# owl-project/owlExaBrick

Measured on AMD Instinct MI355X. Metric: frames/sec at 2048^2 DVR, exajet-like, MI355X, higher is better.
Workload: dtype f32; 1 GPU; c4_exajet (seed 0xe7a0003 procedural AMR, scale 1.0): 640512000 cells / 1251000 bricks / 13349488 regions, 2048x2048 DVR, dt 0.5, alpha ramp, gradient shading on, space skipping on, frameID 0; tiling=16x16 tiles interleaved over 1 GPU(s)

## Files before the change

### owlexabrick_amd/csrc/exa_device.h

```cpp
#pragma once
#include "../../include/exa_hip.h"
#include <hip/hip_runtime.h>

#include <vector>

#ifndef EXA_MARCH_WAVES
#define EXA_MARCH_WAVES 6
#endif
#ifndef EXA_ROPE_WAVES
#define EXA_ROPE_WAVES 7
#endif
#ifndef EXA_MULTI_WAVES
#define EXA_MULTI_WAVES 6
#endif
#ifndef EXA_PREPASS_WAVES
#define EXA_PREPASS_WAVES 4
#endif
#ifndef EXA_IL2_WAVES
#define EXA_IL2_WAVES 5
#endif
#ifndef EXA_IL34_WAVES
#define EXA_IL34_WAVES 4
#endif
#ifndef EXA_PREPASS_ISO_WAVES
#define EXA_PREPASS_ISO_WAVES 4
#endif
#ifndef EXA_AO_ISO_WAVES
#define EXA_AO_ISO_WAVES 6
#endif
#ifndef EXA_EMPTY_CELLS
#define EXA_EMPTY_CELLS 0
#endif
#ifndef EXA_BASIS_FORM
#define EXA_BASIS_FORM 0
#endif
namespace exa {

struct alignas(64) BvhNode {
  float4 q0, q1, q2;
  int32_t child0, child1, pad0, pad1;
};
static_assert(sizeof(BvhNode) == 64, "node must be one 64-byte line");

struct alignas(16) RegionInfo {
  int32_t listBegin;
  int32_t listSize;
  float   finestLevelCellWidth;
  int32_t firstBrick;
};

struct alignas(16) KdNodeDev {
  float    split;
  uint32_t word;
  int32_t  left, right;
};
static_assert(sizeof(KdNodeDev) == 16, "kd node = one 16-byte load");

struct alignas(16) RopeLeaf {
  float    lo[3], hi0;
  float    hi1, hi2;
  uint32_t rec;
  uint32_t flags;
  int32_t  rope[6];
  int32_t  region;
  int32_t  pad;
};
static_assert(sizeof(RopeLeaf) == 64, "rope leaf = four 16-byte loads");

struct alignas(16) RegionRec {
  float   lo[3], hi0;
  float   hi1, hi2, finestLevelCellWidth; int32_t firstBrick;
  int32_t listBegin, listSize, pad0, pad1;
};
static_assert(sizeof(RegionRec) == 48, "region record = three 16-byte loads");

struct DeviceScene {
  const int4       *bricks;
  const int32_t    *leafList;
  const int4       *leafHdr;
  const float      *scalars;
  const RegionInfo *regionInfo;
  const float2     *valueRange;
  const float      *domain;
  unsigned long long channelOffset[EXA_MAX_CHANNELS];
  uint32_t numRegions;
  uint32_t numInternal;
};

#ifndef EXA_KD_STACK
#define EXA_KD_STACK 4
#endif
#ifndef EXA_KD_STACK_MULTI
#define EXA_KD_STACK_MULTI 3
#endif
#ifndef EXA_ROPE_QUEUE
#define EXA_ROPE_QUEUE 5
#endif
#ifndef EXA_ROPE_QUEUE_MULTI
#define EXA_ROPE_QUEUE_MULTI 5
#endif
#ifndef EXA_SEG_QUEUE
#define EXA_SEG_QUEUE 4
#endif
enum { kKdStackEntries = EXA_KD_STACK, kKdStackMultiEntries = EXA_KD_STACK_MULTI };
enum { kTile = 16, kTilePixels = 256, kStackDepth = 32, kKdStack = EXA_KD_STACK, kKdStackMulti = EXA_KD_STACK_MULTI, kSegQueue = EXA_SEG_QUEUE,
       kRopeQueue = EXA_ROPE_QUEUE, kRopeQueueMulti = EXA_ROPE_QUEUE_MULTI,
       kKdBlock = 256,
       kWideSegCap = 256,
       kWalkProbeBits = 15, kWalkProbeSize = 1 << kWalkProbeBits };

enum StatSlot { ST_SEGMENTS, ST_SAMPLE_EVALS, ST_SAMPLES, ST_BRICK_VISITS, ST_CORNER_LOADS,
                ST_ISO_SEGMENTS, ST_ISO_EVALS, ST_NODES,
                ST_W_BRICK, ST_L_BRICK, ST_W_FINAL, ST_L_FINAL, ST_W_NODE, ST_L_NODE, ST_W_LEAF, ST_L_LEAF,
                ST_KD_MISMATCH,
                ST_T_BRICK, ST_T_FINAL, ST_T_WALK, ST_T_SEG, ST_T_OTHER,
                ST_RESTARTS, ST_UNION, ST_PROBE_OVERFLOW, ST_WAVE_ITERS, ST_TILE_ITERS,
                ST_ROPE_LEAVES,
                ST_COUNT };

struct alignas(16) AoRecord { float4 posFd, ngAmb, baseRnd; uint32_t slot, pad0, pad1, pad2; };
static_assert(sizeof(AoRecord) == 64, "AO record = four 16-byte stores");

struct RenderArgs {
  DeviceScene        sc;
  const BvhNode     *volNodes;
  const BvhNode     *isoNodes;
  const KdNodeDev   *kdNodes;
  const KdNodeDev   *kdMarchNodes;
  int32_t            kdMarchRoot;
  uint32_t           leafBeginBits, leafSizeBits;
  const RegionRec   *regionRec;
  const RopeLeaf    *ropeLeaves;
  const KdNodeDev   *ropeNodes;
  int32_t            ropeRoot;
  int32_t            ropeFastDiv;
  int32_t            ropeAddr32;
  int32_t            kdRoot;
  int32_t            kdIsoRoot;
  float              kdLo[3], kdHi[3];
  const BvhNode     *meshNodes;
  const float       *meshVerts;
  const int32_t     *meshTris;
  int32_t            numTris;
  const BvhNode     *streamNodes;
  const float       *traces;
  int32_t            numStreamPrims;
  int32_t            tracerChannels[3], numTraces, numTimesteps, timestep;
  float              steplen;
  float              worldLo[3], worldHi[3];
  ExaHipFrameState   fs;
  ExaHipParams       p;
  const float4      *xf;
  const float       *cellsIl;
  int32_t            il32;
  int32_t            mul24;
  int32_t            addr32;
  float              invDtPow2;
  int32_t            fastSampler;
  float              tfFracMagic;
  int32_t            numXfChannels;
  int32_t            W, H, tilesX, tilesY;
  int32_t            rank, world;
  const int32_t     *tileMap;
  uint32_t          *color;
  int32_t            colorRowMajor;
  float4            *accum;
  float4            *surf;
  float4            *pixOut;
  uint32_t          *surfRnd;
  unsigned long long *stats;
  int32_t           *errorFlag;
  int32_t            debugPixel;
  const int32_t     *wideTileMap;
  float4            *wideSegs;
  uint32_t          *walkProbe;
  AoRecord          *aoRecs;
  uint32_t          *aoCount;
  uint32_t          *aoKeys;
  uint32_t          *aoHist;
  uint32_t          *aoOrder;
  uint8_t           *aoHit;
  uint32_t           aoBins;
  uint32_t          *tileCostPre;
  uint32_t          *tileCost;
};

struct SampleArgs {
  const int4        *leafHdr;
  const float       *scalars;
  const KdNodeDev   *kdNodes;
  const RegionRec   *regionRec;
  int32_t            kdRoot;
  int32_t            maxSteps;
  float              kdLo[3], kdHi[3];
  int32_t           *errorFlag;
  int32_t            world;
  int32_t            normalized;
  float              fill;
  ExaHipFrameState   fs;
  int32_t            numChannels;
  unsigned long long fieldOffset[EXA_MAX_CHANNELS];
  const float       *points;
  unsigned long long count;
  float             *values, *gradients;
  int32_t           *status;
  float              lo[3], step[3];
  int32_t            box0[3], box1[3];
  unsigned long long patchesX, patchesY, numPatches;
  unsigned long long strideY, strideZ;
  float             *out;
};
enum { kSamplePatchShapes = 4 };

hipError_t buildLbvhTopologyDevice(const float *boxes, uint32_t numPrims, BvhNode *nodes, int32_t *levelIds,
                                   std::vector<uint32_t> &internalNodesPerDepth, hipStream_t s);

#define EXA_FORM_LAUNCHERS                                                                                              \
  hipError_t launchRender(const RenderArgs &a, int numBlocks, bool grad, bool iso, bool stats, hipStream_t s);          \
  hipError_t launchSurfacePrepassKd(const RenderArgs &a, int numBlocks, bool stats, hipStream_t s);                     \
   \
  hipError_t launchAoRaysKd(const RenderArgs &a, int numBlocks, hipStream_t s);                                         \
  hipError_t launchCompositeKd(const RenderArgs &a, int numBlocks, hipStream_t s);                                      \
  hipError_t launchRenderKd(const RenderArgs &a, int numBlocks, bool grad, bool fast, bool surf,                        \
                            int stats , hipStream_t s);                                 \
                                                                    \
  hipError_t launchRenderKdRope(const RenderArgs &a, int numBlocks, bool grad, bool fast, bool surf,                    \
                                int stats, hipStream_t s);                                                              \
  hipError_t launchRenderKdWide(const RenderArgs &a, int numTiles, int lanesPerRay, bool grad, bool fast, bool surf,    \
                                hipStream_t s);                                                                         \
                          \
  hipError_t launchComputeTraces(const RenderArgs &a, float *traces, int count, hipStream_t s);                        \
    \
  hipError_t launchSamplePoints(const SampleArgs &a, bool grad, hipStream_t s);                                      \
  hipError_t launchSampleGrid(const SampleArgs &a, int shape, bool uniform, hipStream_t s);
namespace form0 { EXA_FORM_LAUNCHERS }
namespace form1 { EXA_FORM_LAUNCHERS }
namespace form0e { EXA_FORM_LAUNCHERS }
#undef EXA_FORM_LAUNCHERS

hipError_t launchVolumeActivity(const DeviceScene &sc, const ExaHipFrameState &fs, const ExaHipParams &p,
                                const float4 *xf, uint8_t *active, float tfFracMagic, hipStream_t s);
hipError_t launchIsoActivity(const DeviceScene &sc, const ExaHipFrameState &fs, uint8_t *active, hipStream_t s);
hipError_t launchRefit(BvhNode *nodes, const int32_t *nodeIds, int count, const float *domain,
                       const uint8_t *active, hipStream_t s);
hipError_t launchKdRefit(KdNodeDev *nodes, KdNodeDev *marchNodes, const int32_t *nodeIds, int count, const uint8_t *active, int which, hipStream_t s);
hipError_t launchRopeActivity(RopeLeaf *leaves, uint32_t numRegions, const uint8_t *active, int which, uint32_t *activeCount, hipStream_t s);
hipError_t launchPermuteBricks(const float *src, float *dst, const uint32_t *srcBegin, const uint32_t *dstBegin, int4 *bricks,
                               unsigned long long numBricks, int4 *leafHdr, const int32_t *leafList, unsigned long long leafListSize,
                               unsigned long long totalCells, int numFields, hipStream_t s);
hipError_t launchInterleave(const DeviceScene &sc, unsigned long long totalCells, int nch, float *out, hipStream_t s);
hipError_t launchUntile(const uint32_t *gathered, unsigned long long shardStride, int world,
                        int W, int H, uint32_t *out, hipStream_t s);
hipError_t launchProfileMarker(int tag, hipStream_t s);

}
```

### owlexabrick_amd/csrc/exa_kernels.hip

```cpp
#include "exa_device.h"
#include <cfloat>

#if EXA_BASIS_FORM == 0 && EXA_EMPTY_CELLS
#define EXA_FORM_NS form0e
#elif EXA_BASIS_FORM == 0
#define EXA_FORM_NS form0
#elif EXA_BASIS_FORM == 1 && EXA_EMPTY_CELLS
#error "empty cells are a per-corner property: the per-axis association (EXA_BASIS_FORM 1) does not apply"
#elif EXA_BASIS_FORM == 1
#define EXA_FORM_NS form1
#else
#error "EXA_BASIS_FORM is 0 (source order) or 1 (per-axis association with fused multiply-adds)"
#endif
#define EXA_F1 (EXA_BASIS_FORM == 1)
#ifndef EXA_TU_ROPE
#define EXA_TU_ROPE 0
#endif
#ifndef EXA_TU_SAMPLE
#define EXA_TU_SAMPLE 0
#endif
namespace exa {
namespace EXA_FORM_NS {

struct V3 { float x, y, z; };
// ... 1595 lines not shown
  if (!ISO_ONLY && C.a->numTris > 0) traceMeshes(C, ray, prd);
  if (!ISO_ONLY && withContourPlanes) {
    for (int i = 0; i < EXA_MAX_CONTOUR_PLANES; ++i)
      if (C.a->fs.contour[i].enabled) {
        auto find = [&](V3 pos) { return kdFindRegion(C, pos, stackF, qRegion, qT); };
        const SurfaceHit c = traceContourRay(C, ray, mk(C.a->fs.contour[i].normal), C.a->fs.contour[i].offset,
                                             C.a->fs.contour[i].channel, find);
        if (c.primID == EXA_PRIMID_PLANE && c.t_hit < prd.t_hit) prd = c;
      }
  }
  if (!ISO_ONLY && C.a->numStreamPrims > 0) traceStreamlines(C, ray, prd);
  bool activeIso = false;
  for (int i = 0; i < EXA_MAX_ISO_SURFACES; i++) activeIso |= (C.a->fs.iso[i].enabled != 0);
  if (activeIso) {
    const SurfaceHit isoPRD = traceIsoRayKd(C, ray, 0.f, stackF, qRegion, qT, !withContourPlanes);
    if (isoPRD.primID == EXA_PRIMID_ISOSURFACE && isoPRD.t_hit < prd.t_hit) prd = isoPRD;
  }
}

template <int STATS, bool ISO_ONLY, bool AO_DEFER>
__global__ __launch_bounds__(kKdBlock, (ISO_ONLY ? EXA_PREPASS_ISO_WAVES : EXA_PREPASS_WAVES)) void surfacePrepassKdKernel(const RenderArgs a)
{
  extern __shared__ __attribute__((aligned(16))) unsigned char smem[];
  float4 *xfLds = reinterpret_cast<float4 *>(smem);
  unsigned char *sp0 = smem + size_t(a.numXfChannels) * EXA_NUM_XF_VALUES * sizeof(float4);
  int *stackRef = reinterpret_cast<int *>(sp0);
  float *stackF = reinterpret_cast<float *>(sp0 + size_t(kKdStackEntries) * kKdBlock * 4) + threadIdx.x;
  int *qRegion = reinterpret_cast<int *>(sp0 + size_t(kKdStack) * kKdBlock * 12) + threadIdx.x;
  float *qT = reinterpret_cast<float *>(sp0 + size_t(kKdStack) * kKdBlock * 12 + size_t(kSegQueue) * kKdBlock * 4) + threadIdx.x;
  for (int i = threadIdx.x; i < a.numXfChannels * EXA_NUM_XF_VALUES; i += kKdBlock) xfLds[i] = a.xf[i];
  __syncthreads();

  Ctx<STATS> C;
  C.a = &a;
  C.xfLds = xfLds;
  C.stack = stackRef + threadIdx.x;
  C.guardTripped = false;
  C.fastSampler = a.fastSampler != 0 && STATS != 1;
  if (STATS) for (int i = 0; i < ST_COUNT; i++) C.st[i] = 0;

  const int wavesPerBlock = kKdBlock / 64;
  const int gwave = blockIdx.x * wavesPerBlock + (threadIdx.x >> 6);
  const int tile = a.tileMap[gwave >> 2];
  const int tx = tile % a.tilesX, ty = tile / a.tilesX;
  const int wave = gwave & 3, lane = threadIdx.x & 63;
  const int inX = ((wave & 1) << 3) + laneX(lane), inY = ((wave >> 1) << 3) + laneY(lane);
  const int px = tx * kTile + inX, py = ty * kTile + inY;
  const bool inside = px < a.W && py < a.H && (a.debugPixel < 0 || a.debugPixel == px + a.W * py);

  if (inside) {
    const ExaHipFrameState &fs = a.fs;
    const int frameID = fs.frameID;
    Lcg rnd;
    rnd.init((uint32_t)(frameID * a.W * a.H) + (uint32_t)px, (uint32_t)py);
    const float sx = float(px) + rnd.next();
    const float sy = float(py) + rnd.next();
    Ray ray;
    ray.org = mk(fs.cam_pos);
    ray.dir = normalize((mk(fs.cam_dir00) + sx * mk(fs.cam_dirDu)) + sy * mk(fs.cam_dirDv));
    ray.tmin = 1e-6f; ray.tmax = 1e8f;
    V3 bgColor = mk(0.f, 0.f, 0.f);
    float surface_t_hit = ray.tmax;
    bool deferAo = false;
    AoRecord rec;
    {
      SurfaceHit surface;
      traceSurfacesKd<STATS, ISO_ONLY>(C, ray, surface, true, stackF, qRegion, qT);
      surface_t_hit = surface.t_hit;
      if (surface.primID >= 0 || surface.primID == EXA_PRIMID_ISOSURFACE || surface.primID == EXA_PRIMID_PLANE
          || surface.primID == EXA_PRIMID_STREAMLINE) {
        const bool shade = surface.primID >= 0 || surface.primID == EXA_PRIMID_PLANE || surface.primID == EXA_PRIMID_STREAMLINE
                        || (surface.primID == EXA_PRIMID_ISOSURFACE && a.p.gradientShadingISO);
        if (AO_DEFER && shade && length(surface.Ng) > 0.f && fs.ao.enabled) {
          const V3 isect_pos = ray.org + surface.t_hit * ray.dir;
          rec.posFd = make_float4(isect_pos.x, isect_pos.y, isect_pos.z, fabsf(dot(ray.dir, surface.Ng)));
          rec.ngAmb = make_float4(surface.Ng.x, surface.Ng.y, surface.Ng.z, surface.ambient);
          rec.baseRnd = make_float4(surface.baseColor.x, surface.baseColor.y, surface.baseColor.z, __uint_as_float(rnd.state));
          rnd.next(); rnd.next(); rnd.next(); rnd.next();
          deferAo = true;
        } else if (shade && length(surface.Ng) > 0.f) {
          const float AO_Radius = fs.ao.length;
          const int AO_Samples = (!AO_DEFER && fs.ao.enabled) ? 2 : 0;
          const V3 isect_pos = ray.org + surface.t_hit * ray.dir;
          const V3 wN = surface.Ng;
          const V3 vN = fabsf(wN.x) > fabsf(wN.y) ? normalize(mk(-wN.z, 0.f, wN.x)) : normalize(mk(0.f, wN.z, -wN.y));
          const V3 uN = cross(vN, wN);
          int hitCnt = 0;
          for (int i = 0; i < AO_Samples; ++i) {
            const float u1 = rnd.next(), u2 = rnd.next();
            const float r = sqrtf(u1);
            const float theta = 2.f * 3.14159265358979323846f * u2;
            const V3 sp = mk(r * cosf(theta), r * sinf(theta), sqrtf(1.f - u1));
            Ray ao_ray;
            ao_ray.org = isect_pos;
            ao_ray.dir = normalize((sp.x * uN + sp.y * vN) + sp.z * wN);
            ao_ray.tmin = 1e-4f; ao_ray.tmax = AO_Radius;
            SurfaceHit ao;
            traceSurfacesKd<STATS, ISO_ONLY>(C, ao_ray, ao, false, stackF, qRegion, qT);
            if (ao.primID >= 0 || ao.primID == EXA_PRIMID_ISOSURFACE || ao.primID == EXA_PRIMID_PLANE
                || ao.primID == EXA_PRIMID_STREAMLINE) hitCnt++;
          }
          const float shadow = (!AO_DEFER && fs.ao.enabled) ? (float)hitCnt / AO_Samples : 0.f;
          const float fd = fabsf(dot(ray.dir, surface.Ng));
          const float ns = 1.f - shadow;
          bgColor = mk(surface.ambient + surface.baseColor.x * fd * ns,
                       surface.ambient + surface.baseColor.y * fd * ns,
                       surface.ambient + surface.baseColor.z * fd * ns);
        } else {
          bgColor = surface.baseColor;
        }
      }
    }
    const size_t slot = (a.world == 1) ? size_t(px) + size_t(a.W) * py
                                       : size_t(tile / a.world) * kTilePixels + (inY * kTile + inX);
    a.surf[slot] = make_float4(bgColor.x, bgColor.y, bgColor.z, surface_t_hit);
    a.surfRnd[slot] = rnd.state;
    if (AO_DEFER) {
      const unsigned long long m = __ballot(deferAo);
      if (m) {
        const int lane_ = threadIdx.x & 63;
        const int leader = __ffsll((long long)m) - 1;
        unsigned base = 0;
        if (lane_ == leader) base = atomicAdd(a.aoCount, (unsigned)__popcll(m));
        base = (unsigned)__shfl((int)base, leader, 64);
        if (deferAo) {
          rec.slot = (uint32_t)slot; rec.pad0 = rec.pad1 = rec.pad2 = 0;
          a.aoRecs[base + (unsigned)__popcll(m & ((1ull << lane_) - 1ull))] = rec;
        }
      }
    }
  }

  if (a.tileCostPre) {
    unsigned v = inside ? C.isoSteps : 0u;
    for (int off = 32; off > 0; off >>= 1) v = max(v, (unsigned)__shfl_down((int)v, off, 64));
    if ((threadIdx.x & 63) == 0) atomicMax(&a.tileCostPre[tile], v);
  }
  if (C.guardTripped) atomicExch(a.errorFlag, 1);
  if (STATS) {
    for (int i = 0; i < ST_COUNT; i++) {
      unsigned long long v = inside ? C.st[i] : 0ull;
      for (int off = 32; off > 0; off >>= 1) v += __shfl_down(v, off, 64);
      if ((threadIdx.x & 63) == 0 && v) atomicAdd(&a.stats[i], v);
    }
  }
}

__device__ __forceinline__ Ray aoRayOf(const ExaHipFrameState &fs, const float4 posFd, const float4 ngAmb, const float4 baseRnd, unsigned j)
{
  Lcg rnd;
  rnd.state = __float_as_uint(baseRnd.w);
  if (j & 1u) { rnd.next(); rnd.next(); }
  const V3 wN = mk(ngAmb.x, ngAmb.y, ngAmb.z);
  const V3 vN = fabsf(wN.x) > fabsf(wN.y) ? normalize(mk(-wN.z, 0.f, wN.x)) : normalize(mk(0.f, wN.z, -wN.y));
  const V3 uN = cross(vN, wN);
  const float u1 = rnd.next(), u2 = rnd.next();
  const float rr = sqrtf(u1);
  const float theta = 2.f * 3.14159265358979323846f * u2;
  const V3 sp = mk(rr * cosf(theta), rr * sinf(theta), sqrtf(1.f - u1));
  Ray ao_ray;
  ao_ray.org = mk(posFd.x, posFd.y, posFd.z);
  ao_ray.dir = normalize((sp.x * uN + sp.y * vN) + sp.z * wN);
  ao_ray.tmin = 1e-4f; ao_ray.tmax = fs.ao.length;
  return ao_ray;
}

enum { kAoDirClasses = 24, kAoCellShift = 5 };
__device__ __forceinline__ uint32_t aoRayKey(const RenderArgs &a, uint32_t slot, V3 d)
{
  const float ax = fabsf(d.x), ay = fabsf(d.y), az = fabsf(d.z);
  const uint32_t dom = (ax >= ay && ax >= az) ? 0u : (ay >= az ? 1u : 2u);
  const uint32_t oct = (d.x < 0.f ? 1u : 0u) | (d.y < 0.f ? 2u : 0u) | (d.z < 0.f ? 4u : 0u);
  uint32_t cell;
  if (a.world == 1) {
    const uint32_t px = slot % (uint32_t)a.W, py = slot / (uint32_t)a.W;
    cell = (py >> kAoCellShift) * (((uint32_t)a.W + 31u) >> kAoCellShift) + (px >> kAoCellShift);
  } else {
    cell = slot >> 10;
  }
  return cell * kAoDirClasses + oct * 3u + dom;
}
#if !EXA_TU_ROPE
__global__ __launch_bounds__(256) void aoKeyKernel(const RenderArgs a)
{
  const unsigned numRays = 2u * a.aoCount[0];
  for (unsigned j = blockIdx.x * 256u + threadIdx.x; j < numRays; j += gridDim.x * 256u) {
    const AoRecord *r = a.aoRecs + (j >> 1);
    const Ray ray = aoRayOf(a.fs, r->posFd, r->ngAmb, r->baseRnd, j);
    const uint32_t key = min(aoRayKey(a, r->slot, ray.dir), a.aoBins - 1u);
    a.aoKeys[j] = key;
    atomicAdd(&a.aoHist[key], 1u);
  }
}
__global__ __launch_bounds__(1024) void aoScanKernel(uint32_t *hist, uint32_t numBins)
{
  __shared__ uint32_t part[1024];
  const uint32_t per = (numBins + 1023u) / 1024u;
  const uint32_t b0 = min(threadIdx.x * per, numBins), b1 = min(b0 + per, numBins);
  uint32_t sum = 0;
  for (uint32_t b = b0; b < b1; b++) sum += hist[b];
  part[threadIdx.x] = sum;
  __syncthreads();
  for (uint32_t off = 1; off < 1024u; off <<= 1) {
    const uint32_t v = threadIdx.x >= off ? part[threadIdx.x - off] : 0u;
    __syncthreads();
    part[threadIdx.x] += v;
    __syncthreads();
  }
  uint32_t run = part[threadIdx.x] - sum;
  for (uint32_t b = b0; b < b1; b++) { const uint32_t c = hist[b]; hist[b] = run; run += c; }
}
__global__ __launch_bounds__(256) void aoScatterKernel(const RenderArgs a)
{
  const unsigned numRays = 2u * a.aoCount[0];
  for (unsigned j = blockIdx.x * 256u + threadIdx.x; j < numRays; j += gridDim.x * 256u)
    a.aoOrder[atomicAdd(&a.aoHist[a.aoKeys[j]], 1u)] = j;
}
__global__ __launch_bounds__(256) void aoFinalizeKernel(const RenderArgs a)
{
  const unsigned numHits = a.aoCount[0];
  for (unsigned h = blockIdx.x * 256u + threadIdx.x; h < numHits; h += gridDim.x * 256u) {
    const AoRecord *r = a.aoRecs + h;
    const float4 posFd = r->posFd, ngAmb = r->ngAmb, baseRnd = r->baseRnd;
    const uint32_t slot = r->slot;
    const int hitCnt = (int)a.aoHit[2u * h] + (int)a.aoHit[2u * h + 1u];
    const float shadow = (float)hitCnt / 2;
    const float fd = posFd.w;
    const float ns = 1.f - shadow;
    const float t_hit = a.surf[slot].w;
    a.surf[slot] = make_float4(ngAmb.w + baseRnd.x * fd * ns, ngAmb.w + baseRnd.y * fd * ns, ngAmb.w + baseRnd.z * fd * ns, t_hit);
  }
}

#endif

template <bool ISO_ONLY, bool SORTED>
__global__ __launch_bounds__(kKdBlock, (ISO_ONLY ? EXA_AO_ISO_WAVES : EXA_PREPASS_WAVES)) void aoRaysKdKernel(const RenderArgs a)
{
  extern __shared__ __attribute__((aligned(16))) unsigned char smem[];
  float4 *xfLds = reinterpret_cast<float4 *>(smem);
  unsigned char *sp0 = smem + size_t(a.numXfChannels) * EXA_NUM_XF_VALUES * sizeof(float4);
  int *stackRef = reinterpret_cast<int *>(sp0);
  float *stackF = reinterpret_cast<float *>(sp0 + size_t(kKdStackEntries) * kKdBlock * 4) + threadIdx.x;
  int *qRegion = reinterpret_cast<int *>(sp0 + size_t(kKdStack) * kKdBlock * 12) + threadIdx.x;
  float *qT = reinterpret_cast<float *>(sp0 + size_t(kKdStack) * kKdBlock * 12 + size_t(kSegQueue) * kKdBlock * 4) + threadIdx.x;
  for (int i = threadIdx.x; i < a.numXfChannels * EXA_NUM_XF_VALUES; i += kKdBlock) xfLds[i] = a.xf[i];
  __syncthreads();
  Ctx<0> C;
  C.a = &a;
  C.xfLds = xfLds;
  C.stack = stackRef + threadIdx.x;
  C.guardTripped = false;
  C.fastSampler = a.fastSampler != 0;
  const ExaHipFrameState &fs = a.fs;
  const unsigned numRays = 2u * a.aoCount[0];
  for (;;) {
    unsigned base = 0;
    if ((threadIdx.x & 63) == 0) base = atomicAdd(&a.aoCount[2], 64u);
    base = (unsigned)__shfl((int)base, 0, 64);
    if (base >= numRays) break;
    const unsigned k = base + (threadIdx.x & 63);
    const bool live = k < numRays;
    const unsigned j = (SORTED && live) ? a.aoOrder[k] : k;
    int hitFlag = 0;
    float4 posFd = make_float4(0.f, 0.f, 0.f, 0.f), ngAmb = posFd, baseRnd = posFd;
    uint32_t slot = 0;
    if (live) {
      const AoRecord *r = a.aoRecs + (j >> 1);
      posFd = r->posFd; ngAmb = r->ngAmb; baseRnd = r->baseRnd; slot = r->slot;
      const Ray ao_ray = aoRayOf(fs, posFd, ngAmb, baseRnd, j);
      SurfaceHit ao;
      traceSurfacesKd<0, ISO_ONLY>(C, ao_ray, ao, false, stackF, qRegion, qT);
      if (ao.primID >= 0 || ao.primID == EXA_PRIMID_ISOSURFACE || ao.primID == EXA_PRIMID_PLANE
          || ao.primID == EXA_PRIMID_STREAMLINE) hitFlag = 1;
      if (SORTED) a.aoHit[j] = (uint8_t)hitFlag;
    }
    if (SORTED) continue;
    const int other = __shfl_xor(hitFlag, 1, 64);
    if (live && !(j & 1u)) {
      const int hitCnt = hitFlag + other;
      const float shadow = (float)hitCnt / 2;
      const float fd = posFd.w;
      const float ns = 1.f - shadow;
      const float t_hit = a.surf[slot].w;
      a.surf[slot] = make_float4(ngAmb.w + baseRnd.x * fd * ns, ngAmb.w + baseRnd.y * fd * ns, ngAmb.w + baseRnd.z * fd * ns, t_hit);
    }
  }
  if (C.guardTripped) atomicExch(a.errorFlag, 1);
}

constexpr int marchWaves(int MULTI, int STATS, bool SMALL, int NCH, bool ROPE)
{
  return NCH ? (NCH == 2 ? EXA_IL2_WAVES : EXA_IL34_WAVES)
             : (MULTI == 1 ? EXA_MULTI_WAVES
                           : (MULTI ? 5 : ((ROPE && !STATS && SMALL && EXA_BASIS_FORM == 1) ? EXA_ROPE_WAVES : EXA_MARCH_WAVES)));
}

template <bool GRAD, bool FAST, int MULTI, bool SURF, int STATS, bool SMALL, int NCH = 0, bool ROPE = false>
__global__ __launch_bounds__(kKdBlock, marchWaves(MULTI, STATS, SMALL, NCH, ROPE)) void renderFrameKdKernel(const RenderArgs a)
{
  constexpr bool LEAN = marchWaves(MULTI, STATS, SMALL, NCH, ROPE) >= 7;
  constexpr int PACKED_CT = !ROPE ? -1 : (STATS == 1 ? 0 : (SMALL ? 1 : -1));
  const bool packedRec = PACKED_CT < 0 ? a.leafBeginBits != 0 : PACKED_CT != 0;
  static_assert(NCH == 0 || (MULTI == 2 && STATS == 0), "the interleaved march is a multi-channel variant of the shipped kernel");
  constexpr int KSB = MULTI == 1 ? kKdStackMulti : kKdStack;
  constexpr int KS = MULTI == 1 ? kKdStackMultiEntries : kKdStackEntries;
  constexpr int QN = ROPE ? (MULTI == 1 ? kRopeQueueMulti : kRopeQueue) : kSegQueue;
  static_assert(MULTI != 0 || (size_t(EXA_NUM_XF_VALUES) * sizeof(float4) + size_t(kKdBlock) * (ROPE ? QN * 16 : (KSB + QN) * 12))
                                  * marchWaves(MULTI, STATS, SMALL, NCH, ROPE) <= 160 * 1024,
                "LDS per workgroup x waves per SIMD exceeds the CU's 160 KB: shorten the queue or lower the occupancy");
  extern __shared__ __attribute__((aligned(16))) unsigned char smem[];
  float4 *xfLds = reinterpret_cast<float4 *>(smem);
  unsigned char *sp0 = smem + size_t(a.numXfChannels) * EXA_NUM_XF_VALUES * sizeof(float4);
  int *stackRef = reinterpret_cast<int *>(sp0);
  float *stackF = reinterpret_cast<float *>(sp0 + size_t(KS) * kKdBlock * 4) + threadIdx.x;
  unsigned char *q0 = ROPE ? sp0 : sp0 + size_t(KSB) * kKdBlock * 12;
  int *qRegion = reinterpret_cast<int *>(q0) + threadIdx.x;
  float *qT = reinterpret_cast<float *>(q0 + size_t(QN) * kKdBlock * 4) + threadIdx.x;
  float4 *queue4 = reinterpret_cast<float4 *>(sp0) + threadIdx.x;
  for (int i = threadIdx.x; i < a.numXfChannels * EXA_NUM_XF_VALUES; i += kKdBlock) xfLds[i] = a.xf[i];
  __syncthreads();

  Ctx<STATS> C;
  C.a = &a;
  C.xfLds = xfLds;
  C.stack = stackRef + threadIdx.x;
  C.guardTripped = false;
  const unsigned long long clockBegin = clock64();
  if (STATS) for (int i = 0; i < ST_COUNT; i++) C.st[i] = 0;
  __shared__ unsigned long long lapMarks[STATS == 2 ? 8 * (kKdBlock / 64) : 1];
  if (STATS == 2) {
    C.lapMark = lapMarks + 8 * (threadIdx.x >> 6);
    if ((threadIdx.x & 63) == 0) {
      C.lapMark[0] = clock64(); C.lapMark[1] = ST_T_OTHER - ST_T_BRICK;
      for (int i = 2; i < 7; i++) C.lapMark[i] = 0;
    }
  }

  const int wavesPerBlock = kKdBlock / 64;
  const int gwave = blockIdx.x * wavesPerBlock + (threadIdx.x >> 6);
  const int tile = a.tileMap[gwave >> 2];
  const int tx = tile % a.tilesX, ty = tile / a.tilesX;
  const int wave = gwave & 3, lane = threadIdx.x & 63;
  const int inX = ((wave & 1) << 3) + laneX(lane), inY = ((wave >> 1) << 3) + laneY(lane);
  const int px = tx * kTile + inX, py = ty * kTile + inY;
  const bool inside = px < a.W && py < a.H && (a.debugPixel < 0 || a.debugPixel == px + a.W * py);

  if (STATS == 1 && a.walkProbe) C.probe = a.walkProbe + size_t(gwave) * kWalkProbeSize;
  unsigned marchIters = 0;
  if (inside) {
    const ExaHipFrameState &fs = a.fs;
    const int frameID = fs.frameID;
    Lcg rnd;
    rnd.init((uint32_t)(frameID * a.W * a.H) + (uint32_t)px, (uint32_t)py);
    const float sx = float(px) + rnd.next();
    const float sy = float(py) + rnd.next();
    Ray ray;
    ray.org = mk(fs.cam_pos);
    ray.dir = normalize((mk(fs.cam_dir00) + sx * mk(fs.cam_dirDu)) + sy * mk(fs.cam_dirDv));
    ray.tmin = 1e-6f; ray.tmax = 1e8f;
    float surface_t_hit = ray.tmax;
    if (SURF) {
      const size_t slot0 = (a.world == 1) ? size_t(px) + size_t(a.W) * py
                                          : size_t(tile / a.world) * kTilePixels + (inY * kTile + inX);
      surface_t_hit = a.surf[slot0].w;
      rnd.state = a.surfRnd[slot0];
    }
    const float interleavedSamplingOffset = rnd.next();
    ray.tmax = surface_t_hit;
    if (fs.clipBox.enabled) {
      float c0, c1;
      boxTest(ray, mk(fs.clipBox.lo), mk(fs.clipBox.hi), c0, c1);
      ray.tmin = c0; ray.tmax = c1;
    }
    surface_t_hit = ray.tmax;
    ray.org = xfmPoint(fs, ray.org);
    ray.org.x = __int_as_float(__builtin_amdgcn_readfirstlane(__float_as_int(ray.org.x)));
    ray.org.y = __int_as_float(__builtin_amdgcn_readfirstlane(__float_as_int(ray.org.y)));
    ray.org.z = __int_as_float(__builtin_amdgcn_readfirstlane(__float_as_int(ray.org.z)));
    ray.dir = xfmVector(fs, ray.dir);
    const float dt_scale = length(ray.dir);
    ray.dir = normalize(ray.dir);
    ray.tmin = dt_scale * ray.tmin;
    ray.tmax = surface_t_hit * dt_scale;

    Color4 pixelColor; pixelColor.x = pixelColor.y = pixelColor.z = pixelColor.w = 0.f;
    const int numChannels = a.p.numPrimaryChannels;

    KdWalk w;
    w.pk.v = 0;
    {
      Ray whole = ray; whole.tmin = -INFINITY; whole.tmax = INFINITY;
      float r0, r1;
      const bool hit = boxTest(whole, mk(a.kdLo), mk(a.kdHi), r0, r1);
      w.tn = fmaxf(r0, ray.tmin);
      w.tf = fminf(r1, ray.tmax);
      w.tEnd = w.tf;
      w.ref = (hit && w.tn < w.tf) ? (ROPE ? a.ropeRoot : a.kdMarchRoot) : EXA_KD_DONE;
    }
    bool ropeFast = false;
    if (ROPE) ropeFast = a.ropeFastDiv != 0 && !anyLane(!ropeRayInRange(ray));

    float walkTmin = ray.tmin;

    bool haveSeg = false;
    int listBegin = 0, listSize = 0;
    float flcw = 1.f;
    float t1 = 0.f, t_i = 0.f, t_sample = 0.f, actual_dt = 0.f;
    int child = 0, chan = 0;
    int4 hb0 = make_int4(0, 0, 0, 1), hb1 = make_int4(1, 1, 1, 0);
    Basis B;
    B.sumWV = 0.f; B.sumW = 0.f; B.sumD = mk(0.f, 0.f, 0.f); B.sumDC = mk(0.f, 0.f, 0.f);
    float xWV[NCH > 1 ? NCH - 1 : 1];
    V3 xD[NCH > 1 ? NCH - 1 : 1];
#pragma unroll
    for (int c = 0; c < (NCH > 1 ? NCH - 1 : 1); c++) { xWV[c] = 0.f; xD[c] = mk(0.f, 0.f, 0.f); }
    const float *field0 = a.sc.scalars + a.sc.channelOffset[0];
    const float *field = field0;
    float xfRcpRange0 = 0.f, xfRange0 = 0.f;
    if (FAST && !MULTI) {
      xfRange0 = __int_as_float(__builtin_amdgcn_readfirstlane(__float_as_int((fs.xfDomain[0][1] - fs.xfDomain[0][0]) + 1e-20f)));
      xfRcpRange0 = __int_as_float(__builtin_amdgcn_readfirstlane(__float_as_int(__builtin_amdgcn_rcpf(xfRange0))));
    }
    float xfRcpRangeN[NCH ? NCH : 1], xfRangeN[NCH ? NCH : 1];
#pragma unroll
    for (int c = 0; c < (NCH ? NCH : 1); c++) {
      xfRangeN[c] = (FAST && NCH) ? __int_as_float(__builtin_amdgcn_readfirstlane(__float_as_int((fs.xfDomain[c][1] - fs.xfDomain[c][0]) + 1e-20f))) : 0.f;
      xfRcpRangeN[c] = (FAST && NCH) ? __int_as_float(__builtin_amdgcn_readfirstlane(__float_as_int(__builtin_amdgcn_rcpf(xfRangeN[c])))) : 0.f;
    }

    unsigned iter = 0;
    for (;; iter++) {
      if (iter == 0xfffffff0u) { C.guardTripped = true; break; }
      if (anyLane(!haveSeg && w.pk.get(PK_QCOUNT) == 0 && w.ref != EXA_KD_DONE)) {
        C.lap(ST_T_WALK);
        do {
          const bool want = w.pk.get(PK_QCOUNT) < QN && w.ref != EXA_KD_DONE;
          if (want) {
            if (ROPE) ropeStep<STATS, SMALL, QN, LEAN, PACKED_CT>(C, w, walkTmin, a, queue4, ray, ropeFast, interleavedSamplingOffset);
            else kdStep<false, STATS, SMALL, KS>(C, w, walkTmin, a, stackF, qRegion, qT, ray, 0, walkTmin, 1.f, a.kdMarchNodes, a.kdMarchRoot);
          }
        } while (anyLane(!haveSeg && w.pk.get(PK_QCOUNT) == 0 && w.ref != EXA_KD_DONE));
      }
      if (!haveSeg) {
        C.lap(ST_T_SEG);
        const int qc = w.pk.get(PK_QCOUNT);
        if (qc == 0) break;
        const int qh = w.pk.get(PK_QHEAD);
        int region;
        float t0, tiQueued = 0.f;
        if (ROPE) {
          const float4 e = queue4[qh * kKdBlock];
          region = __float_as_int(e.x); t1 = e.y; tiQueued = e.z; t0 = e.w;
        } else {
          region = qRegion[qh * kKdBlock];
          t0 = qT[(2 * qh) * kKdBlock];
          t1 = qT[(2 * qh + 1) * kKdBlock];
        }
        w.pk.template incWrap<QN>(PK_QHEAD);
        w.pk.dec(PK_QCOUNT);
        if (packedRec) {
          const unsigned d = (unsigned)region;
          listBegin = (int)(d & ((1u << a.leafBeginBits) - 1u));
          listSize = (int)((d >> a.leafBeginBits) & ((1u << a.leafSizeBits) - 1u)) + 1;
          flcw = __int_as_float((127 + (int)(d >> (a.leafBeginBits + a.leafSizeBits))) << 23);
        } else {
          const RegionInfo ri = a.sc.regionInfo[region];
          listBegin = ri.listBegin; listSize = ri.listSize;
          flcw = ri.finestLevelCellWidth;
        }
        C.count(ST_SEGMENTS);
        haveSeg = true;
        w.pk.setBit(PK_NEEDHDR);
        if (ROPE && packedRec)
          t_i = tiQueued;
        else if (a.invDtPow2 != 0.f)
          t_i = firstSampleTPow2(t0, a.p.dt * flcw, a.invDtPow2 * __int_as_float(0x7f000000 - __float_as_int(flcw)), interleavedSamplingOffset);
        else
          t_i = firstSampleT(t0, a.p.dt * flcw, interleavedSamplingOffset);
        {
          const float t_next = fminf(t_i, t1);
          t_sample = 0.5f * (fminf(t1, t_next) + t0);
          actual_dt = t_next - t0;
        }
        C.count(ST_SAMPLE_EVALS);
      }

      C.lap(ST_T_BRICK);
      C.phase(ST_W_BRICK);
      if (listSize > 1 || w.pk.get(PK_NEEDHDR)) {
        if (SMALL) {
          const char *hp = reinterpret_cast<const char *>(a.sc.leafHdr) + ((uint32_t)(listBegin + child) << 5);
          hb0 = *reinterpret_cast<const int4 *>(hp); hb1 = *reinterpret_cast<const int4 *>(hp + 16);
        } else {
          const unsigned at = 2u * (unsigned)(listBegin + child);
          hb0 = a.sc.leafHdr[at]; hb1 = a.sc.leafHdr[at + 1u];
        }
        w.pk.clearField(PK_NEEDHDR);
      }
      if (NCH) addBasisFastIl<GRAD, SMALL, (NCH ? NCH : 2)>(B, xWV, xD, hb0, hb1, a.cellsIl, rayAt(ray.org, t_sample, ray.dir));
      else addBasisFast<GRAD, STATS, SMALL>(C, B, hb0, hb1, MULTI ? field : field0, rayAt(ray.org, t_sample, ray.dir));
      child++;
      if (child < listSize) continue;

      C.lap(ST_T_FINAL);
      C.phase(ST_W_FINAL);
      if (NCH) {
        if (B.sumW > 1e-20f) {
#pragma unroll
          for (int c = 0; c < NCH; c++) {
            const float wv = c == 0 ? B.sumWV : xWV[c == 0 ? 0 : c - 1];
            const V3 sd = c == 0 ? B.sumD : xD[c == 0 ? 0 : c - 1];
            const float cellValue = fdivExact<FAST>(wv, B.sumW);
            V3 grad = mk(0.f, 0.f, 0.f);
            if (GRAD) grad = gradOf(B.sumW, wv, sd, B.sumDC);
            integrateVolume<FAST, STATS, FAST>(C, ray, pixelColor, actual_dt, cellValue, grad, flcw, c, xfRcpRangeN[c], xfRangeN[c]);
          }
        }
#pragma unroll
        for (int c = 0; c < (NCH > 1 ? NCH - 1 : 1); c++) { xWV[c] = 0.f; xD[c] = mk(0.f, 0.f, 0.f); }
      } else if (B.sumW > 1e-20f) {
        C.count(ST_SAMPLES);
        const float cellValue = fdivExact<FAST>(B.sumWV, B.sumW);
        V3 grad = mk(0.f, 0.f, 0.f);
        if (GRAD) grad = gradOf(B.sumW, B.sumWV, B.sumD, B.sumDC);
        integrateVolume<FAST, STATS, (FAST && !MULTI), LEAN>(C, ray, pixelColor, actual_dt, cellValue, grad, flcw, MULTI ? chan : 0, xfRcpRange0, xfRange0);
      }
      B.sumWV = 0.f; B.sumW = 0.f; B.sumD = mk(0.f, 0.f, 0.f); B.sumDC = mk(0.f, 0.f, 0.f);
      child = 0;
      if (MULTI && !NCH) {
        chan++;
        if (chan < numChannels) {
          field = a.sc.scalars + a.sc.channelOffset[chan];
          C.count(ST_SAMPLE_EVALS);
          continue;
        }
        chan = 0; field = field0;
      }
      if (pixelColor.w >= EXA_TERMINATION_THRESHOLD) {
        pixelColor.x = pixelColor.x * pixelColor.w;
        pixelColor.y = pixelColor.y * pixelColor.w;
        pixelColor.z = pixelColor.z * pixelColor.w;
        pixelColor.w = 1.f;
        break;
      }
      const float t_last = fminf(t_i, t1);
      if (t_last >= t1) {
        haveSeg = false;
        continue;
      }
      t_i += a.p.dt * flcw;
      {
        const float t_next = fminf(t_i, t1);
        t_sample = 0.5f * (fminf(t1, t_next) + t_last);
        actual_dt = t_next - t_last;
      }
      C.count(ST_SAMPLE_EVALS);
    }

    C.lap(ST_T_OTHER);
    marchIters = iter;
    size_t slot, colorSlot;
    {
      unsigned tid = threadIdx.x, bid = blockIdx.x;
      asm volatile("" : "+v"(tid));
      asm volatile("" : "+s"(bid));
      const int lane2 = tid & 63, wave2 = (tid >> 6) & 3;
      const int inX2 = ((wave2 & 1) << 3) + laneX(lane2), inY2 = ((wave2 >> 1) << 3) + laneY(lane2);
      slot = (a.world == 1) ? size_t(tx * kTile + inX2) + size_t(a.W) * (ty * kTile + inY2)
                            : size_t(a.tileMap[(bid * wavesPerBlock + (tid >> 6)) >> 2] / a.world) * kTilePixels + (inY2 * kTile + inX2);
      colorSlot = a.colorRowMajor ? size_t(tx * kTile + inX2) + size_t(a.W) * (ty * kTile + inY2) : slot;
    }
    if (SURF && a.pixOut) {
      a.pixOut[slot] = make_float4(pixelColor.x, pixelColor.y, pixelColor.z, pixelColor.w);
    } else {
    float4 bgColor = make_float4(0.f, 0.f, 0.f, 0.f);
    if (SURF) bgColor = a.surf[slot];
    float cr = pixelColor.w * pixelColor.x + (1.f - pixelColor.w) * bgColor.x;
    float cg = pixelColor.w * pixelColor.y + (1.f - pixelColor.w) * bgColor.y;
    float cb = pixelColor.w * pixelColor.z + (1.f - pixelColor.w) * bgColor.z;
    if (fs.clockScale > 0.f) cr = clockHeat(fs.clockScale, clockBegin);
    if (frameID > 0) {
      const float4 acc = a.accum[slot];
      cr += acc.x; cg += acc.y; cb += acc.z;
    }
    a.accum[slot] = make_float4(cr, cg, cb, 1.f);
    const float div = frameID + 1.f;
    cr = cr / div; cg = cg / div; cb = cb / div;
    a.color[colorSlot] = make_rgba8(linear_to_srgb(cr), linear_to_srgb(cg), linear_to_srgb(cb));
    }
  }

  if (a.tileCost) {
    unsigned v = marchIters;
    for (int off = 32; off > 0; off >>= 1) v = max(v, (unsigned)__shfl_down((int)v, off, 64));
    unsigned bid = blockIdx.x, tid = threadIdx.x;
    asm volatile("" : "+s"(bid));
    asm volatile("" : "+v"(tid));
    if (lane == 0) atomicMax(&a.tileCost[a.tileMap[(bid * wavesPerBlock + (tid >> 6)) >> 2]], v);
  }
  if (C.guardTripped) atomicExch(a.errorFlag, 1);
  if (STATS == 2) {
    if (lane < 5 && C.lapMark[2 + lane]) atomicAdd(&a.stats[ST_T_BRICK + lane], C.lapMark[2 + lane]);
  }
  if (STATS == 1) {
    for (int i = 0; i < ST_COUNT; i++) {
      unsigned long long v = inside ? C.st[i] : 0ull;
      for (int off = 32; off > 0; off >>= 1) v += __shfl_down(v, off, 64);
      if ((threadIdx.x & 63) == 0 && v) atomicAdd(&a.stats[i], v);
    }
    __shared__ unsigned wgMaxIters;
    if (threadIdx.x == 0) wgMaxIters = 0;
    __syncthreads();
    unsigned v = marchIters;
    for (int off = 32; off > 0; off >>= 1) v = max(v, (unsigned)__shfl_down((int)v, off, 64));
    if (lane == 0) atomicMax(&wgMaxIters, v);
    __syncthreads();
    if (lane == 0) atomicAdd(&a.stats[ST_WAVE_ITERS], (unsigned long long)v);
    if (threadIdx.x == 0) atomicAdd(&a.stats[ST_TILE_ITERS], 4ull * wgMaxIters);
  }
}

__device__ __forceinline__ void kdCollectStep(Ctx<0> &C, KdWalk &w, const float winLo, const float winHi, const RenderArgs &a,
                                              float *stackF, const Ray &ray, const KdNodeDev *nodes, const int root,
                                              float4 *out, unsigned &count)
{
  if (w.ref != EXA_KD_EMPTY && !(w.tn < winHi)) { w.ref = EXA_KD_DONE; return; }
  if (w.ref < 0 && w.ref > EXA_KD_DONE) {
    if (w.tn >= winLo && w.tn < w.tf) out[count++] = make_float4(__int_as_float(~w.ref), w.tn, w.tf, 0.f);
    w.ref = EXA_KD_EMPTY;
  }
  if (w.ref == EXA_KD_EMPTY || (w.ref != EXA_KD_DONE && !(w.tf > winLo))) kdPop(C, w, root, stackF, nodes, ray);
#define EXA_KD_POP_LATER() (w.ref = EXA_KD_EMPTY)
  if (w.ref < 0 || !(w.tf > winLo) || !(w.tn < winHi)) return;
  const int4 n = *reinterpret_cast<const int4 *>(nodes + w.ref);
  const float split = __int_as_float(n.x);
  const int axis = n.y & 3;
  const int bits = (n.y >> 2) & 3;
  const float ox = ray.org.x, oy = ray.org.y, oz = ray.org.z, dx = ray.dir.x, dy = ray.dir.y, dz = ray.dir.z;
  float o = axis == 0 ? ox : oy, d = axis == 0 ? dx : dy;
  o = axis == 2 ? oz : o;
  d = axis == 2 ? dz : d;
  if (d == 0.f) {
    if (o < split && (bits & 1)) w.ref = n.z;
    else if (o > split && (bits & 2)) w.ref = n.w;
    else EXA_KD_POP_LATER();
    return;
  }
  const float ts = (split - o) / d;
  const bool nearIsLeft = d > 0.f;
  const int nearRef = nearIsLeft ? n.z : n.w, farRef = nearIsLeft ? n.w : n.z;
  const bool nearAct = (bits & (nearIsLeft ? 1 : 2)) != 0, farAct = (bits & (nearIsLeft ? 2 : 1)) != 0;
  if (ts >= w.tf) {
    if (nearAct) w.ref = nearRef; else EXA_KD_POP_LATER();
  } else if (ts <= w.tn) {
    if (farAct) w.ref = farRef; else EXA_KD_POP_LATER();
  } else if (nearAct) {
    if (farAct) {
      const int head = w.pk.get(PK_SHEAD), count_ = w.pk.get(PK_SCOUNT);
      C.stack[head * kKdBlock] = farRef;
      stackF[(2 * head) * kKdBlock] = ts;
      stackF[(2 * head + 1) * kKdBlock] = w.tf;
      w.pk.template incWrap<kKdStackEntries>(PK_SHEAD);
      if (count_ == kKdStackEntries) w.pk.setBit(PK_DROPPED); else w.pk.inc(PK_SCOUNT);
    }
    w.ref = nearRef;
    w.tf = ts;
  } else if (farAct) {
    w.ref = farRef;
    w.tn = ts;
  } else {
    EXA_KD_POP_LATER();
  }
}
#undef EXA_KD_POP_LATER

template <bool GRAD, bool FAST, bool SURF, int L, bool SMALL>
__global__ __launch_bounds__(kKdBlock, 4) void renderFrameKdWideKernel(const RenderArgs a)
{
  extern __shared__ __attribute__((aligned(16))) unsigned char smem[];
  float4 *xfLds = reinterpret_cast<float4 *>(smem);
  unsigned char *sp0 = smem + size_t(a.numXfChannels) * EXA_NUM_XF_VALUES * sizeof(float4);
  int *stackRef = reinterpret_cast<int *>(sp0);
  float *stackF = reinterpret_cast<float *>(sp0 + size_t(kKdStackEntries) * kKdBlock * 4) + threadIdx.x;
  for (int i = threadIdx.x; i < a.numXfChannels * EXA_NUM_XF_VALUES; i += kKdBlock) xfLds[i] = a.xf[i];
  __syncthreads();

  Ctx<false> C;
  C.a = &a;
  C.xfLds = xfLds;
  C.stack = stackRef + threadIdx.x;
  C.guardTripped = false;
  const unsigned long long clockBegin = clock64();

  __builtin_amdgcn_s_setprio(3);
  const int tile = a.wideTileMap[blockIdx.x / L];
  const int part = blockIdx.x % L;
  const int tx = tile % a.tilesX, ty = tile / a.tilesX;
  const int lane = threadIdx.x & 63, sub = lane & (L - 1), lead = lane & ~(L - 1);
  const bool leader = sub == 0;
  const int r = part * (kTilePixels / L) + (threadIdx.x >> 6) * (64 / L) + lane / L;
  const int inX = (((r >> 6) & 1) << 3) + (r & 7), inY = ((r >> 7) << 3) + ((r >> 3) & 7);
  const int px = tx * kTile + inX, py = ty * kTile + inY;
  const bool inside = px < a.W && py < a.H && (a.debugPixel < 0 || a.debugPixel == px + a.W * py);

  unsigned myVisits = 0;
  if (inside) {
    const ExaHipFrameState &fs = a.fs;
    const int frameID = fs.frameID;
    Lcg rnd;
    rnd.init((uint32_t)(frameID * a.W * a.H) + (uint32_t)px, (uint32_t)py);
    const float sx = float(px) + rnd.next();
    const float sy = float(py) + rnd.next();
    Ray ray;
    ray.org = mk(fs.cam_pos);
    ray.dir = normalize((mk(fs.cam_dir00) + sx * mk(fs.cam_dirDu)) + sy * mk(fs.cam_dirDv));
    ray.tmin = 1e-6f; ray.tmax = 1e8f;
    const size_t slot = (a.world == 1) ? size_t(px) + size_t(a.W) * py
                                       : size_t(tile / a.world) * kTilePixels + (inY * kTile + inX);
    float surface_t_hit = ray.tmax;
    if (SURF) {
      surface_t_hit = a.surf[slot].w;
      rnd.state = a.surfRnd[slot];
    }
    const float interleavedSamplingOffset = rnd.next();
    ray.tmax = surface_t_hit;
    if (fs.clipBox.enabled) {
      float c0, c1;
      boxTest(ray, mk(fs.clipBox.lo), mk(fs.clipBox.hi), c0, c1);
      ray.tmin = c0; ray.tmax = c1;
    }
    surface_t_hit = ray.tmax;
    ray.org = xfmPoint(fs, ray.org);
    ray.dir = xfmVector(fs, ray.dir);
    const float dt_scale = length(ray.dir);
    ray.dir = normalize(ray.dir);
    ray.tmin = dt_scale * ray.tmin;
    ray.tmax = surface_t_hit * dt_scale;

    Color4 pixelColor; pixelColor.x = pixelColor.y = pixelColor.z = pixelColor.w = 0.f;

    float4 *const mySegs = a.wideSegs + (size_t(blockIdx.x / L) * kTilePixels * L + size_t(r) * L + sub) * kWideSegCap;
    unsigned myCount = 0;
    KdWalk w;
    w.pk.v = 0;
    float winLo, winHi;
    {
      Ray whole = ray; whole.tmin = -INFINITY; whole.tmax = INFINITY;
      float r0, r1;
      const bool hit = boxTest(whole, mk(a.kdLo), mk(a.kdHi), r0, r1);
      w.tn = fmaxf(r0, ray.tmin);
      w.tf = fminf(r1, ray.tmax);
      w.tEnd = w.tf;
      w.ref = (hit && w.tn < w.tf) ? a.kdMarchRoot : EXA_KD_DONE;
      const float span = w.tf - w.tn;
      winLo = sub == 0 ? -INFINITY : w.tn + span * (float(sub) / float(L));
      winHi = sub == L - 1 ? INFINITY : w.tn + span * (float(sub + 1) / float(L));
      for (unsigned g = 0;; g++) {
        if (g == 0xfffffff0u) { C.guardTripped = true; break; }
        const bool want = w.ref != EXA_KD_DONE && myCount < kWideSegCap;
        if (!anyLane(want)) break;
        if (want) kdCollectStep(C, w, winLo, winHi, a, stackF, ray, a.kdMarchNodes, a.kdMarchRoot, mySegs, myCount);
      }
    }
    __builtin_amdgcn_fence(__ATOMIC_RELEASE, "wavefront");
    __builtin_amdgcn_fence(__ATOMIC_ACQUIRE, "wavefront");
    float walkTmin = ray.tmin;
    int curWin = 0;
    unsigned curIdx = 0, curCount = (unsigned)__shfl((int)myCount, lead, 64);
    const float4 *curSegs = a.wideSegs + (size_t(blockIdx.x / L) * kTilePixels * L + size_t(r) * L) * kWideSegCap;

    bool haveSeg = false, newStep = false, needHdr = false, mine = false;
    int listBegin = 0, listSize = 0;
    float flcw = 1.f, dtSeg = 0.f;
    float t1 = 0.f, tiBase = 0.f, tlBase = 0.f;
    float t_sample = 0.f, actual_dt = 0.f;
    int child = 0;
    int4 hb0 = make_int4(0, 0, 0, 1), hb1 = make_int4(1, 1, 1, 0);
    Basis B;
    B.sumWV = 0.f; B.sumW = 0.f; B.sumD = mk(0.f, 0.f, 0.f); B.sumDC = mk(0.f, 0.f, 0.f);
    const float *field0 = a.sc.scalars + a.sc.channelOffset[0];

    for (unsigned iter = 0;; iter++) {
      if (iter == 0xfffffff0u) { C.guardTripped = true; break; }
      if (!haveSeg) {
        int region = -1;
        float t0 = 0.f;
        for (;;) {
          if (curIdx >= curCount) {
            const bool mineIsCur = sub == curWin;
            if (__shfl((int)(w.ref != EXA_KD_DONE), lead + curWin, 64)) {
              if (mineIsCur) {
                myCount = 0;
                for (unsigned g = 0; w.ref != EXA_KD_DONE && myCount < kWideSegCap; g++) {
                  if (g == 0xfffffff0u) { C.guardTripped = true; break; }
                  kdCollectStep(C, w, winLo, winHi, a, stackF, ray, a.kdMarchNodes, a.kdMarchRoot, mySegs, myCount);
                }
              }
              __builtin_amdgcn_fence(__ATOMIC_RELEASE, "wavefront");
              __builtin_amdgcn_fence(__ATOMIC_ACQUIRE, "wavefront");
              curIdx = 0;
              curCount = (unsigned)__shfl((int)myCount, lead + curWin, 64);
              continue;
            }
            if (++curWin == L) break;
            curIdx = 0;
            curCount = (unsigned)__shfl((int)myCount, lead + min(curWin, L - 1), 64);
            curSegs += kWideSegCap;
            continue;
          }
          const float4 e = curSegs[curIdx++];
          t0 = fmaxf(walkTmin, e.y);
          if (t0 < e.z) {
            region = __float_as_int(e.x);
            t1 = e.z;
            walkTmin = t1 * (1.0000001f);
            break;
          }
        }
        if (curWin == L) break;
        if (a.leafBeginBits) {
          const unsigned d = (unsigned)region;
          listBegin = (int)(d & ((1u << a.leafBeginBits) - 1u));
          listSize = (int)((d >> a.leafBeginBits) & ((1u << a.leafSizeBits) - 1u)) + 1;
          flcw = __int_as_float((127 + (int)(d >> (a.leafBeginBits + a.leafSizeBits))) << 23);
        } else {
          const RegionInfo ri = a.sc.regionInfo[region];
          listBegin = ri.listBegin; listSize = ri.listSize;
          flcw = ri.finestLevelCellWidth;
        }
        dtSeg = a.p.dt * flcw;
        tiBase = firstSampleT(t0, dtSeg, interleavedSamplingOffset);
        tlBase = t0;
        haveSeg = true; newStep = true; needHdr = true;
      }
      if (newStep) {
        float ti = tiBase, tl = tlBase, myTn = 0.f, myTl = 0.f;
        bool ex = true;
        mine = false;
#pragma unroll
        for (int s = 0; s < L; s++) {
          const float tn = fminf(ti, t1);
          if (s == sub) { myTn = tn; myTl = tl; mine = ex; }
          ex = ex && tn < t1;
          tl = tn;
          ti = ti + dtSeg;
        }
        t_sample = 0.5f * (fminf(t1, myTn) + myTl);
        actual_dt = myTn - myTl;
        newStep = false;
      }

      if (mine) {
// ... 525 lines not shown
```

Baseline: 59.11 frames/s.

## Switch directly to next queued segment at segment end in rope march

When a segment's sampling finishes and the segment queue has entries, the march loop now pops the next queued segment in place. It decodes the packed leaf record and sets up the first sample directly, instead of falling back through the haveSeg=false path. The queue entry is loaded from LDS before the final integration so its latency overlaps that work. This is meant to cut loop-iteration overhead and the wave divergence that comes from going through the generic segment-fetch branch. In exchange it adds a speculative LDS load and more code in the hot loop, which may raise register pressure.

After: 58.96 frames/s. About the same (-0.2%).

```diff
diff --git a/owlexabrick_amd/csrc/exa_device.h b/owlexabrick_amd/csrc/exa_device.h
--- a/owlexabrick_amd/csrc/exa_device.h
+++ b/owlexabrick_amd/csrc/exa_device.h
@@ -27,6 +27,9 @@
 #endif
 #ifndef EXA_AO_ISO_WAVES
 #define EXA_AO_ISO_WAVES 6
+#endif
+#ifndef EXA_SEG_SWITCH
+#define EXA_SEG_SWITCH 1
 #endif
 #ifndef EXA_EMPTY_CELLS
 #define EXA_EMPTY_CELLS 0
diff --git a/owlexabrick_amd/csrc/exa_kernels.hip b/owlexabrick_amd/csrc/exa_kernels.hip
--- a/owlexabrick_amd/csrc/exa_kernels.hip
+++ b/owlexabrick_amd/csrc/exa_kernels.hip
@@ -1921,6 +1921,9 @@
   constexpr bool LEAN = marchWaves(MULTI, STATS, SMALL, NCH, ROPE) >= 7;
   constexpr int PACKED_CT = !ROPE ? -1 : (STATS == 1 ? 0 : (SMALL ? 1 : -1));
   const bool packedRec = PACKED_CT < 0 ? a.leafBeginBits != 0 : PACKED_CT != 0;
+#if EXA_SEG_SWITCH
+  constexpr bool SEG_SWITCH = ROPE && PACKED_CT != 0;
+#endif
   static_assert(NCH == 0 || (MULTI == 2 && STATS == 0), "the interleaved march is a multi-channel variant of the shipped kernel");
   constexpr int KSB = MULTI == 1 ? kKdStackMulti : kKdStack;
   constexpr int KS = MULTI == 1 ? kKdStackMultiEntries : kKdStackEntries;
@@ -2124,6 +2127,10 @@
 
       C.lap(ST_T_FINAL);
       C.phase(ST_W_FINAL);
+#if EXA_SEG_SWITCH
+      float4 qNext = make_float4(0.f, 0.f, 0.f, 0.f);
+      if (SEG_SWITCH) qNext = queue4[w.pk.get(PK_QHEAD) * kKdBlock];
+#endif
       if (NCH) {
         if (B.sumW > 1e-20f) {
 #pragma unroll
@@ -2163,11 +2170,40 @@
         pixelColor.w = 1.f;
         break;
       }
+#if EXA_SEG_SWITCH
+      const float t_last = t_i;
+      if (t_i >= t1) {
+        if (SEG_SWITCH && packedRec && w.pk.get(PK_QCOUNT) != 0) {
+          C.lap(ST_T_SEG);
+          w.pk.template incWrap<QN>(PK_QHEAD);
+          w.pk.dec(PK_QCOUNT);
+          const unsigned d = (unsigned)__float_as_int(qNext.x);
+          listBegin = (int)(d & ((1u << a.leafBeginBits) - 1u));
+          listSize = (int)((d >> a.leafBeginBits) & ((1u << a.leafSizeBits) - 1u)) + 1;
+          flcw = __int_as_float((127 + (int)(d >> (a.leafBeginBits + a.leafSizeBits))) << 23);
+          C.count(ST_SEGMENTS);
+          w.pk.setBit(PK_NEEDHDR);
+          t1 = qNext.y; t_i = qNext.z;
+          {
+            const float t0 = qNext.w;
+            const float t_next = fminf(t_i, t1);
+            t_sample = 0.5f * (fminf(t1, t_next) + t0);
+            actual_dt = t_next - t0;
+          }
+          C.count(ST_SAMPLE_EVALS);
+          C.lap(ST_T_FINAL);
+          continue;
+        }
+        haveSeg = false;
+        continue;
+      }
+#else
       const float t_last = fminf(t_i, t1);
       if (t_last >= t1) {
         haveSeg = false;
         continue;
       }
+#endif
       t_i += a.p.dt * flcw;
       {
         const float t_next = fminf(t_i, t1);
```
